# Farmadupe/vid_dup_finder_lib

Hardware: AMD Instinct MI355X
Metric: hash-pairs/sec all-pairs Hamming (search(), tolerance 0.35) [+ frames/sec DCT-hash in 'summary.hash_summary'] (higher is better)
Workload: dtype fp4 e2m1 ({0,1}) x fp4 -> f32 accumulate (exact half-integers < 2^11)

## Files before the change

### vid_dup_finder_lib_amd/csrc/api.cpp

```cpp
#include <algorithm>
#include <chrono>
#include <cmath>
#include <cstdio>
#include <cstdlib>
#include <cstring>
#include <memory>
#include <numeric>

#include "host_sort.h"
#include "vdf_ctx.h"

namespace {
thread_local std::string g_create_error;
inline double now_ms() { return std::chrono::duration<double, std::milli>(std::chrono::steady_clock::now().time_since_epoch()).count(); }
}

vdf_ctx::~vdf_ctx()
{
    if (!subs.empty() || !workers.empty()) vdf_impl::destroy_multi(this);
    if (copy_pool) vdf_impl::destroy_copy_pool(this);
    for (auto &kv : axis_tables) {
        kv.second->start.release(); kv.second->size.release(); kv.second->w.release();
        delete kv.second;
    }
    for (auto &kv : mfma_tables) {
        kv.second->operand.release(); kv.second->bias.release(); kv.second->meta.release();
        delete kv.second;
    }
    for (auto &kv : box_tables) {
        kv.second->blob.release(); kv.second->entries.release();
        delete kv.second;
    }
    DevBuf *all[] = {&row_lo, &row_hi, &tile_lo, &tile_hi, &tile_first, &tile_count, &tile_offset, &counters,
                     &hits, &perm, &matched, &exp_cols, &exp_rows, &pop_cols, &pop_rows, &cand, &group_cmin, &group_offset, &group_blocks, &up_hashes,
                     &up_dur, &up_ref_hashes, &up_ref_dur, &small, &frames, &frames2, &out_hashes, &out_hashes2, &out_dc,
                     &out_dc2, &cos_table, &crops, &crop_desc, &crop_tables, &crop_desc2, &crop_tables2, &crop_work, &sort_scratch, &sort_scratch_pub, &hits2, &hit_bitmaps, &bitmap_gather,
                     &out_zero, &out_zero2, &up_zero, &variant_hashes, &align_plan, &align_scratch, &align_up};
    for (DevBuf *b : all) b->release();
    for (PinBuf &b : pin) b.release();
    for (PinBuf &b : pin_out) b.release();
    pin_small.release();
    pin_ctrl.release();
    pin_crops.release();
    pin_desc.release();
    host_hits.buf.release();
    if (ev0) (void)hipEventDestroy(ev0);
    if (ev1) (void)hipEventDestroy(ev1);
    if (ev_mid) (void)hipEventDestroy(ev_mid);
    if (ev_wait) (void)hipEventDestroy(ev_wait);
    for (hipEvent_t e : ev_copy) if (e) (void)hipEventDestroy(e);
    for (hipEvent_t e : ev_done) if (e) (void)hipEventDestroy(e);
    if (copy_stream) (void)hipStreamDestroy(copy_stream);
    if (stream) (void)hipStreamDestroy(stream);
}

namespace vdf_impl {

// ... 89 lines not shown
    L.prune_step = 16;
    if (ctx->mfma_prune_step >= 0) {
        L.prune_step = ctx->mfma_prune_step;
    } else {
        for (int st = 6; st <= 14; st++) {
            const double bits = 64.0 * (st + 1);
            if (bits / 2 - 2.0 * std::sqrt(bits) >= (double)tol_int + 1) { L.prune_step = st; break; }
        }
    }
    if (mfma) L.prune_step = L.prune_step <= 6 ? 6 : L.prune_step <= 8 ? 8 : L.prune_step <= 10 ? 10 : L.prune_step <= 14 ? L.prune_step : 16;
    else L.prune_step = L.prune_step <= 6 ? 6 : L.prune_step <= 10 ? 10 : L.prune_step <= 12 ? 12 : 16;
    if (mfma) {
        L.group_size = std::min<uint32_t>(ctx->mfma_group, L.n_row_tiles);
        L.n_groups = (L.n_row_tiles + L.group_size - 1) / L.group_size;
        if (L.n_groups > 1024) return fail(ctx, VDF_E_INVAL, "too many row-tile groups");
        VDF_HIP(ctx, ctx->group_cmin.reserve((size_t)L.n_groups * 4));
        VDF_HIP(ctx, ctx->group_offset.reserve(((size_t)L.n_groups + 1) * 4));
        VDF_HIP(ctx, ctx->group_blocks.reserve((size_t)L.n_groups * 4));
        L.group_blocks = ctx->group_blocks.as<uint32_t>();
        L.group_cmin = ctx->group_cmin.as<uint32_t>();
        L.group_offset = ctx->group_offset.as<uint32_t>();
        const uint32_t k_steps = (uint32_t)(L.prune_step < 15 ? L.prune_step + 1 : 16);
        const uint32_t col_pad = (uint32_t)((n_cols + vdf::kMfmaRowPad - 1) / vdf::kMfmaRowPad * vdf::kMfmaRowPad) + vdf::kMfmaColPad;
        VDF_HIP(ctx, ctx->exp_cols.reserve((size_t)col_pad * 512));
        VDF_HIP(ctx, ctx->pop_cols.reserve((size_t)col_pad * 12));
        const ExpOwner want_owner{d_col_hashes, n_cols, k_steps, ctx->exp_cols.p};
        const bool reuse = ctx->pinned_db == d_col_hashes && ctx->pinned_n == n_cols && ctx->exp_owner == want_owner;
        if (!reuse) {
            ctx->exp_owner = ExpOwner{};
            VDF_HIP(ctx, vdf::launch_expand_fp4(L.col_hashes, (uint32_t)n_cols, col_pad, ctx->exp_cols.p, k_steps,
                                                ctx->pop_cols.as<float>(), stream));
            ctx->exp_owner = want_owner;
        }
        L.col_exp = ctx->exp_cols.p;
        L.col_pop3 = ctx->pop_cols.as<float>();
        L.col_pad = col_pad;
        if (d_row_hashes == d_col_hashes) {
            L.row_exp = ctx->exp_cols.p;
            L.row_pop3 = L.col_pop3;
            L.row_pad = col_pad;
        } else {
            const uint32_t row_pad = (uint32_t)((padded_rows + 127) / 128 * 128);
            VDF_HIP(ctx, ctx->exp_rows.reserve((size_t)row_pad * 512));
            VDF_HIP(ctx, ctx->pop_rows.reserve((size_t)row_pad * 12));
            VDF_HIP(ctx, vdf::launch_expand_fp4(L.row_hashes, (uint32_t)n_rows, row_pad, ctx->exp_rows.p, k_steps,
                                                ctx->pop_rows.as<float>(), stream));
            L.row_exp = ctx->exp_rows.p;
            L.row_pop3 = ctx->pop_rows.as<float>();
            L.row_pad = row_pad;
        }
    }
    const unsigned long long init[8] = {0, 0, 0, 0, 0xFFFFFFFFull, 0, 0, 0};
    const bool pin_ok = ctx->pin_small.reserve(kPinSmallBytes) && ctx->pin_small.pinned;
    uint64_t spec = std::min<uint64_t>(capacity, std::max<uint64_t>(ctx->hits_guess + ctx->hits_guess / 4 + 1024, 8192));
    if (!pin_ok || spec * sizeof(vdf_hit) > kPinSmallBytes) spec = 0;
    const bool spec_sort = spec && ctx->hits_guess >= kSpecSortHits;
    if (spec_sort) VDF_HIP(ctx, hipMemsetAsync(ctx->hits.p, 0xFF, (size_t)spec * sizeof(vdf_hit), stream));
    const bool adapt_refs = mode == 1 && mfma && ctx->mfma_chunk_cols == 0;
    if (adapt_refs && ctx->refs_hint_cols == n_cols && ctx->refs_hint_rows == n_rows && ctx->refs_hint_chunk) L.chunk_cols = ctx->refs_hint_chunk;
    if (!ctx->pin_ctrl.reserve(256)) return fail(ctx, VDF_E_OOM, "pinned staging");
    unsigned long long *pre = ctx->pin_ctrl.as<unsigned long long>() + 8;
    uint32_t total_tiles = 0;
    unsigned long long unsorted = 0, admitted = 0;
    for (int pass = 0;; pass++) {
        VDF_HIP(ctx, hipMemcpyAsync(ctx->counters.p, init, sizeof init, hipMemcpyHostToDevice, stream));
        VDF_HIP(ctx, vdf::launch_windows_tiles(mode, d_col_dur, (uint32_t)n_cols, d_row_dur, d_row_perm, (uint32_t)n_rows,
                                               row_begin, row_end, shard_index, shard_count, L, stream));
        VDF_HIP(ctx, hipMemcpyAsync(pre, L.counters, 64, hipMemcpyDeviceToHost, stream));
        VDF_HIP(ctx, hipMemcpyAsync(pre + 8, mfma ? L.group_offset + L.n_groups : L.tile_offset + L.n_row_tiles, 4,
                                    hipMemcpyDeviceToHost, stream));
        VDF_HIP(ctx, hipMemcpyAsync(pre + 9, L.tile_offset + L.n_row_tiles, 4, hipMemcpyDeviceToHost, stream));
        VDF_HIP(ctx, hipStreamSynchronize(stream));
// ... 2117 lines not shown
```

### vid_dup_finder_lib_amd/csrc/hamming.hip

```cpp
#include <algorithm>

#include "vdf_internal.h"

namespace vdf {

constexpr uint32_t kMaxBlocksPerLaunch = 4u << 20;

typedef const __attribute__((address_space(4))) uint32_t *const_u32_ptr;

__device__ __forceinline__ uint32_t sat_u32(double x)
{
    if (!(x == x)) return 0u;
    if (x <= 0.0) return 0u;
    if (x >= 4294967295.0) return 0xFFFFFFFFu;
    return (uint32_t)x;
}

__device__ __forceinline__ uint32_t partition_point_lt(const uint32_t *__restrict__ d, uint32_t n, uint32_t v)
{
    uint32_t lo = 0, hi = n;
    while (lo < hi) {
        uint32_t mid = lo + ((hi - lo) >> 1);
        if (d[mid] < v) lo = mid + 1; else hi = mid;
    }
// ... 255 lines not shown
#pragma unroll
            for (int k = 1; k < R; k++) m = min(m, d[k]);
        }
        if (__builtin_amdgcn_ballot_w64(m <= tol) != 0ull) {
            bool col_ok = true;
            if (matched) col_ok = ((((const_u32_ptr)(uintptr_t)matched)[c >> 5] >> (c & 31)) & 1u) == 0u;
            if (col_ok) {
#pragma unroll
                for (int k = 0; k < R; k++)
                    wave_append_hits(d[k] <= tol && c >= rlo[k] && c < rhi[k], rid[k], c, hits, capacity, counters, overflow_row);
            }
        }
    }
    if (threadIdx.x == 0) atomicAdd(&counters[1], (unsigned long long)(c_end - c_begin) * TILE_ROWS);
    if (CHKW < 32 && lane == 0 && n_early) atomicAdd(&counters[3], (unsigned long long)n_early * (64u * R));
}

typedef int v8i __attribute__((ext_vector_type(8)));
typedef int v4i __attribute__((ext_vector_type(4)));
typedef float v16f __attribute__((ext_vector_type(16)));

__global__ __launch_bounds__(256) void expand_fp4_kernel(const uint32_t *__restrict__ packed, uint32_t n,
                                                        uint32_t n_pad, uint4 *__restrict__ expanded,
                                                        uint32_t k_steps, float *__restrict__ pop,
                                                        float *__restrict__ popk, float *__restrict__ popkT)
{
    for (size_t idx = (size_t)blockIdx.x * 256 + threadIdx.x; idx < (size_t)n_pad * 32;
         idx += (size_t)gridDim.x * 256) {
    const uint32_t hsh = (uint32_t)(idx >> 5), dw = (uint32_t)idx & 31u;
    uint4 out = {0u, 0u, 0u, 0u};
    uint32_t w = 0;
    if (hsh < n) {
        w = packed[idx];
        uint32_t o[4];
#pragma unroll
        for (int j = 0; j < 4; j++) {
            uint32_t x = (w >> (8 * j)) & 0xFFu;
            x = (x | (x << 12)) & 0x000F000Fu;
            x = (x | (x << 6)) & 0x03030303u;
            x = (x | (x << 3)) & 0x11111111u;
            o[j] = x << 1;
        }
        out = make_uint4(o[0], o[1], o[2], o[3]);
    }
    expanded[idx] = out;
    if (pop) {
        uint32_t pc = (uint32_t)__builtin_popcount(w), pk = (dw & 15u) < k_steps ? pc : 0u;
#pragma unroll
        for (int o = 16; o > 0; o >>= 1) { pc += (uint32_t)__shfl_xor((int)pc, o, 32); pk += (uint32_t)__shfl_xor((int)pk, o, 32); }
        if (dw == 0) {
            pop[hsh] = (float)pc;
            popk[hsh] = (float)pk;
            popkT[(size_t)(hsh >> 7) * 128 + (hsh & 31u) * 4 + ((hsh >> 5) & 3u)] = (float)pk;
        }
    }
    }
}

template <int N>
struct IntC { static constexpr int value = N; };
template <int I, int N, class F>
__device__ __forceinline__ void static_for(F &&f)
{
    if constexpr (I < N) {
        f(IntC<I>{});
        static_for<I + 1, N>(f);
    }
}

struct CandEntry {
    uint32_t row_base;
    uint32_t col;
    uint32_t mask;
    uint32_t pad;
};

__global__ __launch_bounds__(256) void resolve_candidates_kernel(
    const CandEntry *__restrict__ cand, const unsigned long long *__restrict__ cand_head, uint32_t cand_capacity,
// ... 68 lines not shown
            if (bal == 0ull) continue;
            const uint32_t cnt = (uint32_t)__builtin_popcountll(bal);
            if (staged + cnt > kStage) flush();
            if (hit) {
                vdf_hit hp; hp.row = row_index_base + src; hp.col = ce.col;
                s_stage[wave][staged + __builtin_amdgcn_mbcnt_hi((uint32_t)(bal >> 32), __builtin_amdgcn_mbcnt_lo((uint32_t)bal, 0u))] = hp;
            }
            staged += cnt;
        }
    }
    flush();
}

template <int CHK, int WAVES>
__global__ __launch_bounds__(64 * WAVES, 2) void hamming_mfma2_kernel(
    const uint4 *__restrict__ row_exp, const uint32_t *__restrict__ row_perm, uint32_t n_rows,
    uint32_t row_index_base, const uint4 *__restrict__ col_exp, const uint32_t *__restrict__ row_lo,
    const uint32_t *__restrict__ row_hi, const uint32_t *__restrict__ tile_lo, const uint32_t *__restrict__ tile_hi,
    const uint32_t *__restrict__ tile_first, const uint32_t *__restrict__ tile_count,
    const uint32_t *__restrict__ group_offset, const uint32_t *__restrict__ group_cmin, uint32_t n_groups,
    uint32_t group_size, uint32_t shard_index, uint32_t shard_count, uint32_t n_row_tiles, uint32_t chunk_cols,
    uint32_t tol, const uint32_t *__restrict__ matched, int self_mode, vdf_hit *__restrict__ hits,
    unsigned long long capacity, unsigned long long *__restrict__ counters, uint32_t *__restrict__ overflow_row,
    uint32_t block_base, const float *__restrict__ row_pop3, uint32_t row_pad, const float *__restrict__ col_pop3,
    uint32_t col_pad, CandEntry *__restrict__ cand, uint32_t cand_capacity, unsigned long long *__restrict__ cand_head)
{
    constexpr int K = CHK < 15 ? CHK + 1 : 16;
    constexpr bool kRowcLds = K > 13;
    constexpr uint32_t kSub = WAVES >= 8 ? 4 : 2;
    constexpr uint32_t kColStep = 32 * kSub;
    constexpr int NBLK = 2 * (int)kSub;
    constexpr int NM = NBLK * K;
    constexpr int P = (K == 16 && WAVES >= 8) ? 2 : 4, NB = P + 1;
    constexpr uint32_t kTileRows = 64 * WAVES;
    constexpr int kDmaPerWave = (int)(kColStep * 32 / (64 * WAVES));
    constexpr int kDmaEvery = NM / kDmaPerWave;
    static_assert(kDmaEvery >= 2, "stage too short for its DMA pieces");
    constexpr int kTestAt = 2;
    static_assert(K >= kTestAt + 4, "block too short to hide the previous block's test");
    const uint32_t bid = blockIdx.x + block_base;
    __shared__ __attribute__((aligned(16))) uint4 s_b0[kColStep * 32];
    __shared__ __attribute__((aligned(16))) uint4 s_b1[kColStep * 32];
    const uint32_t tid = threadIdx.x, lane = tid & 63, g = lane >> 5, c31 = lane & 31;
    const uint32_t wave = (uint32_t)__builtin_amdgcn_readfirstlane((int)(tid >> 6));

    const_u32_ptr goff = (const_u32_ptr)(uintptr_t)group_offset;
    uint32_t gl = 0, gh = n_groups;
    while (gh - gl > 1) {
        const uint32_t mid = (gl + gh) >> 1;
        if (goff[mid] <= bid) gl = mid; else gh = mid;
    }
    const uint32_t idx = bid - goff[gl];
    const uint32_t per_group = (group_size + shard_count - 1) / shard_count;
    const uint32_t g0 = gl * group_size;
    const uint32_t t0 = g0 + (shard_index + shard_count - g0 % shard_count) % shard_count;
    const uint32_t t = t0 + (idx % per_group) * shard_count;
    const uint32_t chunk = ((const_u32_ptr)(uintptr_t)group_cmin)[gl] + idx / per_group;
    if (t >= n_row_tiles || t >= g0 + group_size) return;
    {
        const uint32_t f = ((const_u32_ptr)(uintptr_t)tile_first)[t], cnt = ((const_u32_ptr)(uintptr_t)tile_count)[t];
        if (chunk < f || chunk >= f + cnt) return;
    }
    const uint32_t t_lo = ((const_u32_ptr)(uintptr_t)tile_lo)[t];
    const uint32_t t_hi = ((const_u32_ptr)(uintptr_t)tile_hi)[t];
    const uint32_t c_begin = max(chunk * chunk_cols, t_lo);
    const uint32_t c_end = min((chunk + 1) * chunk_cols, t_hi);
    if (c_begin >= c_end) return;

    const float tol_f = (float)min(tol, 1024u);
    const float *row_popk = row_pop3 + row_pad;
    const float *col_popkT = col_pop3 + 2 * (size_t)col_pad;
    const uint32_t row0 = t * kTileRows + wave * 64;
    v4i a[2][K];
    const float4 *s_rc = nullptr;
    v16f rowc[2];
    uint32_t live[2];
#pragma unroll
    for (int rt = 0; rt < 2; rt++) {
        live[rt] = 0;
        const uint32_t p = row0 + 32 * rt + c31;
        uint32_t src = p;
        if (p < n_rows && row_perm) src = row_perm[p];
        const uint4 *rp = row_exp + (size_t)src * 32 + 16 * g;
#pragma unroll
        for (int s = 0; s < K; s++) {
            const uint4 v = rp[s];
            a[rt][s] = (v4i){(int)v.x, (int)v.y, (int)v.z, (int)v.w};
        }
#pragma unroll
        for (int r = 0; r < 16; r++) {
            const uint32_t pr = row0 + 32 * rt + (r & 3) + 8 * (r >> 2) + 4 * g;
            const uint32_t sr = (pr < n_rows && row_perm) ? row_perm[pr] : pr;
            rowc[rt][r] = -0.5f * row_popk[sr];
            if (row_hi[pr] > row_lo[pr]) live[rt] |= 1u << r;
        }
    }
    if constexpr (kRowcLds) {
        __shared__ __attribute__((aligned(16))) float4 s_rowc[WAVES * 2 * 2 * 4];
        float4 *mine = s_rowc + ((size_t)wave * 2 * 2 + g) * 4;
        if (c31 == 0) {
#pragma unroll
            for (int rt = 0; rt < 2; rt++)
#pragma unroll
                for (int q = 0; q < 4; q++)
                    mine[rt * 2 * 4 + q] = float4{rowc[rt][4 * q], rowc[rt][4 * q + 1], rowc[rt][4 * q + 2], rowc[rt][4 * q + 3]};
        }
        s_rc = mine;
    }
    const uint32_t cb0 = c_begin & ~(kColStep - 1);
    constexpr uint32_t kColsPerRound = 2 * WAVES;
    constexpr int kOffsets = 32 / kColsPerRound;
    static_assert(kOffsets >= 1 && (kOffsets & (kOffsets - 1)) == 0, "piece addressing");
    const uint32_t c0 = 2 * wave + g;
    uint32_t lane_off[kOffsets];
#pragma unroll
    for (int j = 0; j < kOffsets; j++) lane_off[j] = c0 * 512u + ((((lane & 31) ^ c0) << 4) ^ (16u * kColsPerRound * j));
    auto stage_rsrc = [&](uint32_t cb) __attribute__((always_inline)) {
        return __builtin_amdgcn_make_buffer_rsrc(
            const_cast<char *>(reinterpret_cast<const char *>(col_exp) + (size_t)cb * 512), 0, kColStep * 512u, 0x00020000);
    };
    auto load_piece = [&](__amdgpu_buffer_rsrc_t rs, uint4 *dst, int i) __attribute__((always_inline)) {
        auto *lds = (__attribute__((address_space(3))) void *)&dst[64 * WAVES * i + 64 * wave];
        const int voff = (int)lane_off[i & (kOffsets - 1)], soff = (int)(512u * kColsPerRound * (uint32_t)i);
        __builtin_amdgcn_raw_ptr_buffer_load_lds(rs, lds, 16, voff, soff, 0, 0);
    };
    auto load_thr = [&](uint32_t cb, float (&out)[kSub]) __attribute__((always_inline)) {
        const float *q = col_popkT + (size_t)(cb >> 7) * 128 + c31 * 4 + ((cb >> 5) & 3u);
        if constexpr (kSub == 4) {
            const float4 v = *reinterpret_cast<const float4 *>(q);
            out[0] = v.x; out[1] = v.y; out[2] = v.z; out[3] = v.w;
        } else {
            const float2 v = *reinterpret_cast<const float2 *>(q);
            out[0] = v.x; out[1] = v.y;
        }
    };

    v16f acc[2] = {v16f{}, v16f{}};
    if constexpr (kRowcLds) acc[0] = rowc[0];
    uint32_t n_early = 0;
    float thr[kSub], thr_next[kSub];

    constexpr uint32_t kCandChunk = 8, kCandChunkMax = 512;
    uint32_t q_chunk = kCandChunk, q_taken = 0;
    unsigned long long q_next = 0, q_end = 0;
    auto emit = [&](const v16f &c, float thrv, uint32_t live_rows, uint32_t rows_first, uint32_t col_first) __attribute__((always_inline)) {
        uint32_t mask = 0;
#pragma unroll
        for (int r = 0; r < 16; r++) mask |= (c[r] >= thrv) ? (1u << r) : 0u;
        mask &= live_rows;
        const uint32_t j = col_first + c31;
        if (j < c_begin || j >= c_end) mask = 0;
        const unsigned long long bal = __builtin_amdgcn_ballot_w64(mask != 0u);
        if (bal == 0ull) return;
        const uint32_t need = (uint32_t)__builtin_popcountll(bal);
        if (q_next + need > q_end) {
            if (q_taken >= 2) q_chunk = min(2u * q_chunk, kCandChunkMax);
            q_taken++;
            const uint32_t take = max((need + kCandChunk - 1) / kCandChunk * kCandChunk, q_chunk);
            unsigned long long base = 0;
            if (lane == 0) base = atomicAdd(cand_head, (unsigned long long)take);
            q_next = ((unsigned long long)(uint32_t)__builtin_amdgcn_readfirstlane((int)(base >> 32)) << 32) |
                     (uint32_t)__builtin_amdgcn_readfirstlane((int)(uint32_t)base);
            q_end = q_next + take;
        }
        const unsigned long long slot = q_next + __builtin_amdgcn_mbcnt_hi((uint32_t)(bal >> 32), __builtin_amdgcn_mbcnt_lo((uint32_t)bal, 0u));
        if (mask != 0u) {
            if (slot < cand_capacity) {
                CandEntry ce; ce.row_base = rows_first + 4 * g; ce.col = j; ce.mask = mask; ce.pad = 0;
                *reinterpret_cast<uint4 *>(&cand[slot]) = *reinterpret_cast<const uint4 *>(&ce);
            } else {
                const uint32_t p = rows_first + 4 * g + (uint32_t)(__builtin_ctz(mask) & 3) + 8 * (uint32_t)(__builtin_ctz(mask) >> 2);
                if (p < n_rows) atomicMin(overflow_row, row_index_base + (row_perm ? row_perm[p] : p));
            }
        }
        q_next += need;
    };

    auto run_stage = [&](uint32_t cb, const uint4 *cur, uint4 *nxt) __attribute__((always_inline)) {
        const uint32_t cb_next = cb + kColStep < c_end ? cb + kColStep : cb;
        const __amdgpu_buffer_rsrc_t rs_next = stage_rsrc(cb_next);
        load_thr(cb_next, thr_next);
        uint32_t flags = 0;
        uint4 fq[NB];
        auto frag = [&](int i) __attribute__((always_inline)) {
            const uint32_t sub = (uint32_t)((i / K) >> 1), s = (uint32_t)(i % K);
            return cur[((32u * sub + c31) << 5) | ((s + 16u * g) ^ c31)];
        };
#pragma unroll
        for (int i = 0; i < P; i++) fq[i] = frag(i);
        __builtin_amdgcn_sched_barrier(0);
        float m0 = 0.f, m1 = 0.f, m2 = 0.f, m3 = 0.f, m4 = 0.f, m5 = 0.f;
        static_for<0, NM>([&](auto ic) __attribute__((always_inline)) {
            constexpr int i = decltype(ic)::value;
            constexpr int blk = i / K, s = i % K, rt = blk & 1;
            const uint4 bv = fq[i % NB];
            const v8i b = {(int)bv.x, (int)bv.y, (int)bv.z, (int)bv.w, 0, 0, 0, 0};
            const v8i ar = {a[rt][s].x, a[rt][s].y, a[rt][s].z, a[rt][s].w, 0, 0, 0, 0};
            if constexpr (s == 0 && !kRowcLds) acc[rt] = __builtin_amdgcn_mfma_scale_f32_32x32x64_f8f6f4(ar, b, rowc[rt], 4, 4, 0, 0, 0, 0);
            else acc[rt] = __builtin_amdgcn_mfma_scale_f32_32x32x64_f8f6f4(ar, b, acc[rt], 4, 4, 0, 0, 0, 0);
            if constexpr (i + P < NM) fq[(i + P) % NB] = frag(i + P);
            if constexpr ((i % kDmaEvery) == 1 && (i / kDmaEvery) < kDmaPerWave) load_piece(rs_next, nxt, i / kDmaEvery);
            if constexpr (blk >= 1) {
                const v16f &c = acc[rt ^ 1];
                if constexpr (s == kTestAt) {
                    m0 = fmaxf(fmaxf(c[0], c[1]), c[2]); m1 = fmaxf(fmaxf(c[3], c[4]), c[5]); m2 = fmaxf(fmaxf(c[6], c[7]), c[8]);
                } else if constexpr (s == kTestAt + 1) {
                    m3 = fmaxf(fmaxf(c[9], c[10]), c[11]); m4 = fmaxf(fmaxf(c[12], c[13]), c[14]);
                } else if constexpr (s == kTestAt + 2) {
                    m5 = fmaxf(fmaxf(m0, m1), m2); m3 = fmaxf(fmaxf(m3, m4), c[15]);
                } else if constexpr (s == kTestAt + 3) {
                    if (__builtin_amdgcn_ballot_w64(fmaxf(m5, m3) >= thr[(blk - 1) >> 1]) != 0ull) {
                        flags |= 1u << (blk - 1);
                        emit(c, thr[(blk - 1) >> 1], live[rt ^ 1], row0 + 32u * (uint32_t)(rt ^ 1), cb + 32u * (uint32_t)((blk - 1) >> 1));
                    }
                }
            }
            if constexpr (kRowcLds && s >= kTestAt + 4 && s < kTestAt + 8) {
                constexpr int q = s - (kTestAt + 4);
                const float4 v = s_rc[((rt ^ 1) * 2) * 4 + q];
                acc[rt ^ 1][4 * q + 0] = v.x; acc[rt ^ 1][4 * q + 1] = v.y; acc[rt ^ 1][4 * q + 2] = v.z; acc[rt ^ 1][4 * q + 3] = v.w;
            }
            __builtin_amdgcn_sched_barrier(0);
        });
        {
            const v16f &c = acc[(NBLK - 1) & 1];
            m0 = fmaxf(fmaxf(c[0], c[1]), c[2]); m1 = fmaxf(fmaxf(c[3], c[4]), c[5]); m2 = fmaxf(fmaxf(c[6], c[7]), c[8]);
            m3 = fmaxf(fmaxf(c[9], c[10]), c[11]); m4 = fmaxf(fmaxf(c[12], c[13]), c[14]);
            const float pm = fmaxf(fmaxf(fmaxf(m0, m1), m2), fmaxf(fmaxf(m3, m4), c[15]));
            if (__builtin_amdgcn_ballot_w64(pm >= thr[kSub - 1]) != 0ull) {
                flags |= 1u << (NBLK - 1);
                emit(c, thr[kSub - 1], live[(NBLK - 1) & 1], row0 + 32u * (uint32_t)((NBLK - 1) & 1), cb + 32u * (kSub - 1));
            }
        }
        uint32_t valid = 0;
#pragma unroll
        for (uint32_t sub = 0; sub < kSub; sub++)
            if (cb + 32u * sub < c_end) valid |= 3u << (2 * sub);
        flags &= valid;
        n_early += (uint32_t)__builtin_popcount(valid & ~flags);
        asm volatile("s_waitcnt vmcnt(0)" ::: "memory");
        __syncthreads();
#pragma unroll
        for (uint32_t sub = 0; sub < kSub; sub++) thr[sub] = 0.5f * (thr_next[sub] - tol_f);
    };

#pragma unroll
    for (int i = 0; i < kDmaPerWave; i++) load_piece(stage_rsrc(cb0), s_b0, i);
    load_thr(cb0, thr_next);
#pragma unroll
    for (int rt = 0; rt < 2; rt++)
#pragma unroll
        for (int s = 0; s < K; s++) asm volatile("" ::"v"(a[rt][s]));
    asm volatile("s_waitcnt vmcnt(0)" ::: "memory");
    __syncthreads();
#pragma unroll
    for (uint32_t sub = 0; sub < kSub; sub++) thr[sub] = 0.5f * (thr_next[sub] - tol_f);
    for (uint32_t cb = cb0; cb < c_end; cb += 2 * kColStep) {
        run_stage(cb, s_b0, s_b1);
        if (cb + kColStep >= c_end) break;
        run_stage(cb + kColStep, s_b1, s_b0);
    }
    if (tid == 0) atomicAdd(&counters[1], (unsigned long long)(c_end - c_begin) * kTileRows);
    if (CHK < 15 && lane == 0 && n_early) atomicAdd(&counters[3], (unsigned long long)n_early * (32u * 32u));
}

__global__ __launch_bounds__(256) void hits_mark_incoming_kernel(const vdf_hit *__restrict__ hits, unsigned long long n,
                                                                 uint32_t *__restrict__ has_in)
{
    for (size_t i = (size_t)blockIdx.x * 256 + threadIdx.x; i < n; i += (size_t)gridDim.x * 256) {
        const uint32_t j = hits[i].col;
        if (!((has_in[j >> 5] >> (j & 31)) & 1u)) atomicOr(&has_in[j >> 5], 1u << (j & 31));
    }
}

__global__ __launch_bounds__(256) void hits_mark_covered_kernel(const vdf_hit *__restrict__ hits, unsigned long long n,
                                                                const uint32_t *__restrict__ has_in, uint32_t *__restrict__ covered)
{
    for (size_t i = (size_t)blockIdx.x * 256 + threadIdx.x; i < n; i += (size_t)gridDim.x * 256) {
        const vdf_hit h = hits[i];
// ... 147 lines not shown
                d += __builtin_popcount(v.x ^ hi[4 * q]) + __builtin_popcount(v.y ^ hi[4 * q + 1]) +
                     __builtin_popcount(v.z ^ hi[4 * q + 2]) + __builtin_popcount(v.w ^ hi[4 * q + 3]);
            }
            best = max(best, d);
        }
    }
    best = wave_max(best);
    if ((threadIdx.x & 63) == 0) s_max[threadIdx.x >> 6] = best;
    __syncthreads();
    if (threadIdx.x == 0) out[g] = max(max(s_max[0], s_max[1]), max(s_max[2], s_max[3]));
}

hipError_t launch_group_max_distance(const uint32_t *hashes, const unsigned long long *offsets,
                                     const unsigned long long *members, const uint32_t *ref_hashes,
                                     const long long *ref_index, uint32_t n_groups, uint32_t *out, hipStream_t stream)
{
    if (n_groups == 0) return hipSuccess;
    hipLaunchKernelGGL(group_max_distance_kernel, dim3(n_groups), dim3(256), 0, stream, hashes, offsets, members,
                       ref_hashes, ref_index, out);
    return hipGetLastError();
}

hipError_t launch_expand_fp4(const uint32_t *packed, uint32_t n, uint32_t n_pad, void *expanded, uint32_t k_steps,
                             float *pop3 , hipStream_t stream)
{
    if (n_pad == 0) return hipSuccess;
    if (pop3 && (n_pad % 128u)) return hipErrorInvalidValue;
    const size_t total = (size_t)n_pad * 32;
    hipLaunchKernelGGL(expand_fp4_kernel, dim3((uint32_t)std::min<size_t>((total + 255) / 256, kMaxBlocksPerLaunch)), dim3(256), 0, stream, packed, n, n_pad,
                       reinterpret_cast<uint4 *>(expanded), k_steps, pop3, pop3 ? pop3 + n_pad : nullptr,
                       pop3 ? pop3 + 2 * (size_t)n_pad : nullptr);
    return hipGetLastError();
}

hipError_t launch_hamming_tiles_mfma2(const SearchLaunch &L, uint32_t total_tiles, hipStream_t stream)
{
    if (total_tiles == 0) return hipSuccess;
    if (L.tile_rows != 512 && L.tile_rows != 256) return hipErrorInvalidValue;
    for (uint32_t base = 0; base < total_tiles; base += kMaxBlocksPerLaunch) {
        const uint32_t nb = std::min(kMaxBlocksPerLaunch, total_tiles - base);
#define VDF_MFMA2_LAUNCH(CK, WV)                                                                                    \
    hipLaunchKernelGGL((hamming_mfma2_kernel<CK, WV>), dim3(nb), dim3(64 * WV), 0, stream,                           \
                       reinterpret_cast<const uint4 *>(L.row_exp), L.row_perm, L.n_rows, L.row_index_base,           \
                       reinterpret_cast<const uint4 *>(L.col_exp), L.row_lo, L.row_hi, L.tile_lo, L.tile_hi,         \
                       L.tile_first, L.tile_count, L.group_offset, L.group_cmin, L.n_groups, L.group_size,           \
                       L.shard_index, L.shard_count, L.n_row_tiles, L.chunk_cols, L.tol, L.matched, L.self_mode,     \
                       L.hits, L.capacity, L.counters, L.overflow_row, base, L.row_pop3, L.row_pad, L.col_pop3, L.col_pad,                   \
                       reinterpret_cast<CandEntry *>(L.cand), L.cand_capacity, L.cand_head)
#define VDF_MFMA2_STEPS(WV)                                                                                         \
    switch (L.prune_step) {                                    \
    case 0: case 1: case 2: case 3: case 4: case 5: case 6: VDF_MFMA2_LAUNCH(6, WV); break;                          \
    case 7: case 8: VDF_MFMA2_LAUNCH(8, WV); break;                                                                  \
    case 9: case 10: VDF_MFMA2_LAUNCH(10, WV); break;                                                                \
    case 11: VDF_MFMA2_LAUNCH(11, WV); break;                                                                        \
    case 12: VDF_MFMA2_LAUNCH(12, WV); break;                                                                        \
    case 13: VDF_MFMA2_LAUNCH(13, WV); break;                                                                        \
    case 14: VDF_MFMA2_LAUNCH(14, WV); break;                                                                        \
    default: VDF_MFMA2_LAUNCH(16, WV); break;                                                                        \
    }
        if (L.tile_rows == 512) { VDF_MFMA2_STEPS(8) } else { VDF_MFMA2_STEPS(4) }
#undef VDF_MFMA2_STEPS
#undef VDF_MFMA2_LAUNCH
        hipError_t e = hipGetLastError();
        if (e != hipSuccess) return e;
    }
    return hipSuccess;
}

hipError_t launch_resolve_candidates(const SearchLaunch &L, hipStream_t stream)
{
// ... 8 lines not shown
```

### vid_dup_finder_lib_amd/csrc/vdf_ctx.h

```cpp
#pragma once
#include <condition_variable>
#include <functional>
#include <map>
#include <mutex>
#include <string>
#include <thread>
#include <vector>

#include "resize_tables.h"
#include <atomic>

#include "vdf_internal.h"

inline std::atomic<long long> g_live_device_bytes{0};
inline std::atomic<long long> g_live_pinned_bytes{0};

struct DevBuf {
    void *p = nullptr;
    size_t cap = 0;
    hipError_t reserve(size_t bytes)
    {
        if (bytes <= cap) return hipSuccess;
        release();
        size_t want = bytes + bytes / 8 + 256;
// ... 114 lines not shown
    size_t refs_hint_cols = 0, refs_hint_rows = 0;
    uint32_t refs_hint_chunk = 0;
    bool no_hit_filter = false;
    uint64_t hits_guess = 0;
    PinBuf pin_small;
    std::map<uint32_t, DeviceAxisTable *> axis_tables;
    std::map<uint64_t, DeviceMfmaTable *> mfma_tables;
    std::map<uint64_t, BoxTableSet *> box_tables;
    std::map<uint32_t, bool> axis_symmetric;
    bool no_device_path_order = false;
    bool lb_host_plan = false;
    bool no_lb_fused = false;
    int hash_no_persistent = 0, hash_wgs_per_cu = 3;
    bool hash_wgs_per_cu_set = false;
    uint32_t mfma_chunk_cols = 0, mfma_group = 8192;
    DevBuf group_cmin, group_offset, group_blocks;
    uint32_t mfma_min_wgs = 8192;
    uint64_t cand_scale = 1;
    uint32_t cand_capacity_override = 0;
    uint32_t mfma_self_rows = 512;
    uint32_t mfma_refs_rows = 256;
    int mfma_prune_step = -1;
    int search_backend = 1;
    DevBuf exp_cols, exp_rows, pop_cols, pop_rows, cand;
    size_t cand_dirty = SIZE_MAX;
    int wavestream_knob = 0;
    bool no_rowcrop = false, rowcrop_all = false, no_boxstream = false;
    bool no_smallcrop = false;
    int lb_side_strips = 0;
    int copy_threads = 0;
    size_t host_chunk_bytes = 32u << 20;
    bool host_direct = true;
    bool force_rccl = false;
    bool test_exchange_fail = false;
    bool err_secondary = false;
    int resize_mode = 0;
    struct HostHits {
        PinBuf buf;
        size_t size() const { return buf.cap / sizeof(vdf_hit); }
        bool resize(size_t n) { return buf.reserve(n * sizeof(vdf_hit)); }
        vdf_hit *data() const { return buf.as<vdf_hit>(); }
    } host_hits;
    vdf_impl::CopyPool *copy_pool = nullptr;
    uint64_t r_n_hits = 0;
    uint32_t r_overflow = 0xFFFFFFFFu;
    int r_rc = 0;

// ... 77 lines not shown
```

### vid_dup_finder_lib_amd/csrc/vdf_internal.h

```cpp
#pragma once
#include <hip/hip_runtime.h>
#include <stdint.h>

#include "../../include/vdf.h"
#include "hash_variant.h"
#include "resize_dispatch.h"
#include "windows_plan.h"
#include "align_plan.h"

namespace vdf {

constexpr int kDefaultRowsPerLane = 2;
constexpr uint32_t kDefaultChunkCols = 2048;

struct SearchLaunch {
    const uint32_t *row_hashes;
    const uint32_t *row_perm;
    uint32_t n_rows;
    uint32_t row_index_base;
    const uint32_t *col_hashes;
    uint32_t n_cols;
    const void *row_exp, *col_exp;
    const float *row_pop3 = nullptr, *col_pop3 = nullptr;
    uint32_t row_pad = 0, col_pad = 0;
    void *cand = nullptr;
    uint32_t cand_capacity = 0;
    unsigned long long *cand_head = nullptr;
    uint32_t *row_lo, *row_hi;
    uint32_t *tile_lo, *tile_hi, *tile_first, *tile_count, *tile_offset;
    uint32_t *group_cmin, *group_offset, *group_blocks;
    int prune_step = 16;
    uint32_t shard_index = 0, shard_count = 1;
    uint32_t n_groups, group_size;
    uint32_t n_row_tiles;
    uint32_t tile_rows;
    uint32_t chunk_cols;
    uint32_t tol;
    const uint32_t *matched;
    int self_mode;
    vdf_hit *hits;
    unsigned long long capacity;
    unsigned long long *counters;
    uint32_t *overflow_row;
};

hipError_t launch_windows_tiles(int mode, const uint32_t *col_dur, uint32_t n_cols, const uint32_t *row_dur,
                                const uint32_t *row_perm, uint32_t n_rows, uint32_t row_begin, uint32_t row_end,
                                uint32_t shard_index, uint32_t shard_count, const SearchLaunch &L,
                                hipStream_t stream);
hipError_t launch_hamming_tiles(const SearchLaunch &L, uint32_t total_tiles, hipStream_t stream);
constexpr uint32_t kMfmaRowPad = 512, kMfmaColPad = 128;
hipError_t launch_expand_fp4(const uint32_t *packed, uint32_t n, uint32_t n_pad, void *expanded, uint32_t k_steps,
                             float *pop3, hipStream_t stream);
hipError_t launch_hamming_tiles_mfma2(const SearchLaunch &L, uint32_t total_tiles, hipStream_t stream);
hipError_t launch_resolve_candidates(const SearchLaunch &L, hipStream_t stream);
hipError_t launch_filter_mark_incoming(const vdf_hit *hits, unsigned long long n_hits, uint32_t n_entries, uint32_t *bitmaps, hipStream_t stream);
hipError_t launch_filter_mark_covered(const vdf_hit *hits, unsigned long long n_hits, uint32_t n_entries, uint32_t *bitmaps, hipStream_t stream);
hipError_t launch_filter_compact(const vdf_hit *hits, unsigned long long n_hits, uint32_t n_entries, const uint32_t *bitmaps, vdf_hit *out,
                                 unsigned long long *counter, hipStream_t stream);
hipError_t launch_bitmap_or(uint32_t *dst, const uint32_t *srcs, size_t n_words, uint32_t n_srcs, hipStream_t stream);
hipError_t launch_group_max_distance(const uint32_t *hashes, const unsigned long long *offsets,
                                     const unsigned long long *members, const uint32_t *ref_hashes,
                                     const long long *ref_index, uint32_t n_groups, uint32_t *out, hipStream_t stream);

struct ResizeAxisTable {
    const int32_t *start;
    const int32_t *size;
    const int16_t *w;
    int32_t window;
    int32_t precision;
};

hipError_t launch_resize_generic(const uint8_t *frames, size_t n_clips, uint32_t w, uint32_t h, size_t frame_stride,
                                 size_t clip_stride, ResizeAxisTable th, ResizeAxisTable tv, int need_h, int need_v,
                                 int32_t y_first, int32_t tmp_rows, uint8_t *small, hipStream_t stream);
struct MfmaResizeArgs {
// ... 121 lines not shown
```

Measured before the change: 4669 billion.

## Pack only needed K-steps and popcount into compact per-hash fp4 image

The expanded fp4 hash image now stores only the K slots actually used per half (stride 2K+1) instead of a fixed 32 slots, with the popcount folded into a trailing pad slot rather than separate pop arrays. The MFMA kernel stages the smaller contiguous image into LDS via buffer-to-LDS pieces, reads column popcounts from LDS for thresholds instead of a separate global load, and drops the XOR swizzle addressing. This cuts global-to-LDS traffic and LDS footprint for pruned K, at the risk of LDS bank conflicts from the odd stride.

```diff
diff --git a/vid_dup_finder_lib_amd/csrc/api.cpp b/vid_dup_finder_lib_amd/csrc/api.cpp
--- a/vid_dup_finder_lib_amd/csrc/api.cpp
+++ b/vid_dup_finder_lib_amd/csrc/api.cpp
@@ -32,7 +32,7 @@
         delete kv.second;
     }
     DevBuf *all[] = {&row_lo, &row_hi, &tile_lo, &tile_hi, &tile_first, &tile_count, &tile_offset, &counters,
-                     &hits, &perm, &matched, &exp_cols, &exp_rows, &pop_cols, &pop_rows, &cand, &group_cmin, &group_offset, &group_blocks, &up_hashes,
+                     &hits, &perm, &matched, &exp_cols, &exp_rows, &cand, &group_cmin, &group_offset, &group_blocks, &up_hashes,
                      &up_dur, &up_ref_hashes, &up_ref_dur, &small, &frames, &frames2, &out_hashes, &out_hashes2, &out_dc,
                      &out_dc2, &cos_table, &crops, &crop_desc, &crop_tables, &crop_desc2, &crop_tables2, &crop_work, &sort_scratch, &sort_scratch_pub, &hits2, &hit_bitmaps, &bitmap_gather,
                      &out_zero, &out_zero2, &up_zero, &variant_hashes, &align_plan, &align_scratch, &align_up};
@@ -168,32 +168,23 @@
         L.group_offset = ctx->group_offset.as<uint32_t>();
         const uint32_t k_steps = (uint32_t)(L.prune_step < 15 ? L.prune_step + 1 : 16);
         const uint32_t col_pad = (uint32_t)((n_cols + vdf::kMfmaRowPad - 1) / vdf::kMfmaRowPad * vdf::kMfmaRowPad) + vdf::kMfmaColPad;
-        VDF_HIP(ctx, ctx->exp_cols.reserve((size_t)col_pad * 512));
-        VDF_HIP(ctx, ctx->pop_cols.reserve((size_t)col_pad * 12));
+        const size_t img_bytes = vdf::fp4img::hash_bytes(k_steps);
+        VDF_HIP(ctx, ctx->exp_cols.reserve((size_t)col_pad * img_bytes));
         const ExpOwner want_owner{d_col_hashes, n_cols, k_steps, ctx->exp_cols.p};
         const bool reuse = ctx->pinned_db == d_col_hashes && ctx->pinned_n == n_cols && ctx->exp_owner == want_owner;
         if (!reuse) {
             ctx->exp_owner = ExpOwner{};
-            VDF_HIP(ctx, vdf::launch_expand_fp4(L.col_hashes, (uint32_t)n_cols, col_pad, ctx->exp_cols.p, k_steps,
-                                                ctx->pop_cols.as<float>(), stream));
+            VDF_HIP(ctx, vdf::launch_expand_fp4(L.col_hashes, (uint32_t)n_cols, col_pad, ctx->exp_cols.p, k_steps, stream));
             ctx->exp_owner = want_owner;
         }
         L.col_exp = ctx->exp_cols.p;
-        L.col_pop3 = ctx->pop_cols.as<float>();
-        L.col_pad = col_pad;
         if (d_row_hashes == d_col_hashes) {
             L.row_exp = ctx->exp_cols.p;
-            L.row_pop3 = L.col_pop3;
-            L.row_pad = col_pad;
         } else {
             const uint32_t row_pad = (uint32_t)((padded_rows + 127) / 128 * 128);
-            VDF_HIP(ctx, ctx->exp_rows.reserve((size_t)row_pad * 512));
-            VDF_HIP(ctx, ctx->pop_rows.reserve((size_t)row_pad * 12));
-            VDF_HIP(ctx, vdf::launch_expand_fp4(L.row_hashes, (uint32_t)n_rows, row_pad, ctx->exp_rows.p, k_steps,
-                                                ctx->pop_rows.as<float>(), stream));
+            VDF_HIP(ctx, ctx->exp_rows.reserve((size_t)row_pad * img_bytes));
+            VDF_HIP(ctx, vdf::launch_expand_fp4(L.row_hashes, (uint32_t)n_rows, row_pad, ctx->exp_rows.p, k_steps, stream));
             L.row_exp = ctx->exp_rows.p;
-            L.row_pop3 = ctx->pop_rows.as<float>();
-            L.row_pad = row_pad;
         }
     }
     const unsigned long long init[8] = {0, 0, 0, 0, 0xFFFFFFFFull, 0, 0, 0};
diff --git a/vid_dup_finder_lib_amd/csrc/fp4_image.h b/vid_dup_finder_lib_amd/csrc/fp4_image.h
--- /dev/null
+++ b/vid_dup_finder_lib_amd/csrc/fp4_image.h
@@ -0,0 +1,46 @@
+#pragma once
+#include <stdint.h>
+
+namespace vdf {
+namespace fp4img {
+
+constexpr uint32_t kSlotBytes = 16;
+constexpr uint32_t kPieceSlots = 64;
+constexpr uint32_t kLdsBytes = 160u * 1024u;
+constexpr int kInstantiatedK[8] = {7, 9, 11, 12, 13, 14, 15, 16};
+
+constexpr uint32_t stride(uint32_t K) { return 2 * K + 1; }
+constexpr uint32_t pad_slot(uint32_t K) { return 2 * K; }
+constexpr uint32_t hash_bytes(uint32_t K) { return stride(K) * kSlotBytes; }
+constexpr int slot(uint32_t K, uint32_t dword)
+{
+    return dword < K ? (int)dword : (dword >= 16 && dword < 16 + K) ? (int)(K + dword - 16) : -1;
+}
+constexpr uint32_t dword_of_slot(uint32_t K, uint32_t s) { return s < K ? s : 16 + (s - K); }
+constexpr uint32_t frag_slot(uint32_t K, uint32_t col, uint32_t s, uint32_t g) { return col * stride(K) + s + K * g; }
+
+constexpr uint32_t stage_slots(uint32_t col_step, uint32_t K) { return col_step * stride(K); }
+constexpr uint32_t stage_bytes(uint32_t col_step, uint32_t K) { return stage_slots(col_step, K) * kSlotBytes; }
+constexpr uint32_t pieces(uint32_t col_step, uint32_t K) { return stage_slots(col_step, K) / kPieceSlots; }
+constexpr uint32_t piece_of(uint32_t wave, uint32_t i, uint32_t waves) { return waves * i + wave; }
+constexpr uint32_t wave_pieces(uint32_t col_step, uint32_t K, uint32_t waves, uint32_t wave)
+{
+    return wave < pieces(col_step, K) ? (pieces(col_step, K) - wave + waves - 1) / waves : 0;
+}
+constexpr uint32_t max_wave_pieces(uint32_t col_step, uint32_t K, uint32_t waves) { return wave_pieces(col_step, K, waves, 0); }
+
+constexpr uint32_t col_step(uint32_t waves) { return waves >= 8 ? 128 : 64; }
+constexpr bool rowc_in_lds(uint32_t K) { return K > 13; }
+constexpr uint32_t rowc_bytes(uint32_t K, uint32_t waves) { return rowc_in_lds(K) ? waves * 2 * 2 * 4 * 16 : 0; }
+constexpr uint32_t kernel_lds_bytes(uint32_t K, uint32_t waves) { return 2 * stage_bytes(col_step(waves), K) + rowc_bytes(K, waves); }
+
+constexpr uint8_t kReadB128Groups[4][16] = {
+    {0, 1, 2, 3, 12, 13, 14, 15, 20, 21, 22, 23, 24, 25, 26, 27},
+    {4, 5, 6, 7, 8, 9, 10, 11, 16, 17, 18, 19, 28, 29, 30, 31},
+    {32, 33, 34, 35, 44, 45, 46, 47, 52, 53, 54, 55, 56, 57, 58, 59},
+    {36, 37, 38, 39, 40, 41, 42, 43, 48, 49, 50, 51, 60, 61, 62, 63},
+};
+constexpr uint32_t bank_group(uint32_t byte_addr) { return (byte_addr / 16) % 16; }
+
+}
+}
diff --git a/vid_dup_finder_lib_amd/csrc/hamming.hip b/vid_dup_finder_lib_amd/csrc/hamming.hip
--- a/vid_dup_finder_lib_amd/csrc/hamming.hip
+++ b/vid_dup_finder_lib_amd/csrc/hamming.hip
@@ -301,15 +301,16 @@
 
 __global__ __launch_bounds__(256) void expand_fp4_kernel(const uint32_t *__restrict__ packed, uint32_t n,
                                                         uint32_t n_pad, uint4 *__restrict__ expanded,
-                                                        uint32_t k_steps, float *__restrict__ pop,
-                                                        float *__restrict__ popk, float *__restrict__ popkT)
-{
+                                                        uint32_t k_steps)
+{
+    const uint32_t stride = fp4img::stride(k_steps);
     for (size_t idx = (size_t)blockIdx.x * 256 + threadIdx.x; idx < (size_t)n_pad * 32;
          idx += (size_t)gridDim.x * 256) {
     const uint32_t hsh = (uint32_t)(idx >> 5), dw = (uint32_t)idx & 31u;
+    const int sl = fp4img::slot(k_steps, dw);
     uint4 out = {0u, 0u, 0u, 0u};
     uint32_t w = 0;
-    if (hsh < n) {
+    if (hsh < n && sl >= 0) {
         w = packed[idx];
         uint32_t o[4];
 #pragma unroll
@@ -322,17 +323,12 @@
         }
         out = make_uint4(o[0], o[1], o[2], o[3]);
     }
-    expanded[idx] = out;
-    if (pop) {
-        uint32_t pc = (uint32_t)__builtin_popcount(w), pk = (dw & 15u) < k_steps ? pc : 0u;
-#pragma unroll
-        for (int o = 16; o > 0; o >>= 1) { pc += (uint32_t)__shfl_xor((int)pc, o, 32); pk += (uint32_t)__shfl_xor((int)pk, o, 32); }
-        if (dw == 0) {
-            pop[hsh] = (float)pc;
-            popk[hsh] = (float)pk;
-            popkT[(size_t)(hsh >> 7) * 128 + (hsh & 31u) * 4 + ((hsh >> 5) & 3u)] = (float)pk;
-        }
-    }
+    uint4 *img = expanded + (size_t)hsh * stride;
+    if (sl >= 0) img[sl] = out;
+    uint32_t pk = (uint32_t)__builtin_popcount(w);
+#pragma unroll
+    for (int o = 16; o > 0; o >>= 1) pk += (uint32_t)__shfl_xor((int)pk, o, 32);
+    if (dw == 0) img[fp4img::pad_slot(k_steps)] = make_uint4(__float_as_uint((float)pk), 0u, 0u, 0u);
     }
 }
 
@@ -447,25 +443,26 @@
     uint32_t group_size, uint32_t shard_index, uint32_t shard_count, uint32_t n_row_tiles, uint32_t chunk_cols,
     uint32_t tol, const uint32_t *__restrict__ matched, int self_mode, vdf_hit *__restrict__ hits,
     unsigned long long capacity, unsigned long long *__restrict__ counters, uint32_t *__restrict__ overflow_row,
-    uint32_t block_base, const float *__restrict__ row_pop3, uint32_t row_pad, const float *__restrict__ col_pop3,
-    uint32_t col_pad, CandEntry *__restrict__ cand, uint32_t cand_capacity, unsigned long long *__restrict__ cand_head)
+    uint32_t block_base, CandEntry *__restrict__ cand, uint32_t cand_capacity, unsigned long long *__restrict__ cand_head)
 {
     constexpr int K = CHK < 15 ? CHK + 1 : 16;
-    constexpr bool kRowcLds = K > 13;
-    constexpr uint32_t kSub = WAVES >= 8 ? 4 : 2;
-    constexpr uint32_t kColStep = 32 * kSub;
+    constexpr uint32_t kStride = fp4img::stride(K), kPad = fp4img::pad_slot(K);
+    constexpr bool kRowcLds = fp4img::rowc_in_lds(K);
+    constexpr uint32_t kColStep = fp4img::col_step(WAVES);
+    constexpr uint32_t kSub = kColStep / 32;
     constexpr int NBLK = 2 * (int)kSub;
     constexpr int NM = NBLK * K;
     constexpr int P = (K == 16 && WAVES >= 8) ? 2 : 4, NB = P + 1;
     constexpr uint32_t kTileRows = 64 * WAVES;
-    constexpr int kDmaPerWave = (int)(kColStep * 32 / (64 * WAVES));
+    constexpr uint32_t kPieces = fp4img::pieces(kColStep, K);
+    constexpr int kDmaPerWave = (int)fp4img::max_wave_pieces(kColStep, K, WAVES);
     constexpr int kDmaEvery = NM / kDmaPerWave;
     static_assert(kDmaEvery >= 2, "stage too short for its DMA pieces");
     constexpr int kTestAt = 2;
     static_assert(K >= kTestAt + 4, "block too short to hide the previous block's test");
     const uint32_t bid = blockIdx.x + block_base;
-    __shared__ __attribute__((aligned(16))) uint4 s_b0[kColStep * 32];
-    __shared__ __attribute__((aligned(16))) uint4 s_b1[kColStep * 32];
+    __shared__ __attribute__((aligned(16))) uint4 s_b0[fp4img::stage_slots(kColStep, K)];
+    __shared__ __attribute__((aligned(16))) uint4 s_b1[fp4img::stage_slots(kColStep, K)];
     const uint32_t tid = threadIdx.x, lane = tid & 63, g = lane >> 5, c31 = lane & 31;
     const uint32_t wave = (uint32_t)__builtin_amdgcn_readfirstlane((int)(tid >> 6));
 
@@ -493,8 +490,6 @@
     if (c_begin >= c_end) return;
 
     const float tol_f = (float)min(tol, 1024u);
-    const float *row_popk = row_pop3 + row_pad;
-    const float *col_popkT = col_pop3 + 2 * (size_t)col_pad;
     const uint32_t row0 = t * kTileRows + wave * 64;
     v4i a[2][K];
     const float4 *s_rc = nullptr;
@@ -506,7 +501,7 @@
         const uint32_t p = row0 + 32 * rt + c31;
         uint32_t src = p;
         if (p < n_rows && row_perm) src = row_perm[p];
-        const uint4 *rp = row_exp + (size_t)src * 32 + 16 * g;
+        const uint4 *rp = row_exp + fp4img::frag_slot(K, 0, 0, g) + (size_t)src * kStride;
 #pragma unroll
         for (int s = 0; s < K; s++) {
             const uint4 v = rp[s];
@@ -516,7 +511,7 @@
         for (int r = 0; r < 16; r++) {
             const uint32_t pr = row0 + 32 * rt + (r & 3) + 8 * (r >> 2) + 4 * g;
             const uint32_t sr = (pr < n_rows && row_perm) ? row_perm[pr] : pr;
-            rowc[rt][r] = -0.5f * row_popk[sr];
+            rowc[rt][r] = -0.5f * __uint_as_float(row_exp[(size_t)sr * kStride + kPad].x);
             if (row_hi[pr] > row_lo[pr]) live[rt] |= 1u << r;
         }
     }
@@ -533,37 +528,25 @@
         s_rc = mine;
     }
     const uint32_t cb0 = c_begin & ~(kColStep - 1);
-    constexpr uint32_t kColsPerRound = 2 * WAVES;
-    constexpr int kOffsets = 32 / kColsPerRound;
-    static_assert(kOffsets >= 1 && (kOffsets & (kOffsets - 1)) == 0, "piece addressing");
-    const uint32_t c0 = 2 * wave + g;
-    uint32_t lane_off[kOffsets];
-#pragma unroll
-    for (int j = 0; j < kOffsets; j++) lane_off[j] = c0 * 512u + ((((lane & 31) ^ c0) << 4) ^ (16u * kColsPerRound * j));
     auto stage_rsrc = [&](uint32_t cb) __attribute__((always_inline)) {
         return __builtin_amdgcn_make_buffer_rsrc(
-            const_cast<char *>(reinterpret_cast<const char *>(col_exp) + (size_t)cb * 512), 0, kColStep * 512u, 0x00020000);
+            const_cast<char *>(reinterpret_cast<const char *>(col_exp) + (size_t)cb * fp4img::hash_bytes(K)), 0,
+            fp4img::stage_bytes(kColStep, K), 0x00020000);
     };
-    auto load_piece = [&](__amdgpu_buffer_rsrc_t rs, uint4 *dst, int i) __attribute__((always_inline)) {
-        auto *lds = (__attribute__((address_space(3))) void *)&dst[64 * WAVES * i + 64 * wave];
-        const int voff = (int)lane_off[i & (kOffsets - 1)], soff = (int)(512u * kColsPerRound * (uint32_t)i);
-        __builtin_amdgcn_raw_ptr_buffer_load_lds(rs, lds, 16, voff, soff, 0, 0);
-    };
-    auto load_thr = [&](uint32_t cb, float (&out)[kSub]) __attribute__((always_inline)) {
-        const float *q = col_popkT + (size_t)(cb >> 7) * 128 + c31 * 4 + ((cb >> 5) & 3u);
-        if constexpr (kSub == 4) {
-            const float4 v = *reinterpret_cast<const float4 *>(q);
-            out[0] = v.x; out[1] = v.y; out[2] = v.z; out[3] = v.w;
-        } else {
-            const float2 v = *reinterpret_cast<const float2 *>(q);
-            out[0] = v.x; out[1] = v.y;
+    constexpr uint32_t kPieceBytes = fp4img::kPieceSlots * fp4img::kSlotBytes;
+    const uint32_t lane_off = kPieceBytes * fp4img::piece_of(wave, 0, WAVES) + lane * fp4img::kSlotBytes;
+    auto load_piece = [&](__amdgpu_buffer_rsrc_t rs, uint4 *dst, auto ic) __attribute__((always_inline)) {
+        constexpr uint32_t i = (uint32_t)decltype(ic)::value, first = fp4img::piece_of(0, i, WAVES);
+        if (first + WAVES <= kPieces || wave < kPieces - first) {
+            auto *lds = (__attribute__((address_space(3))) void *)&dst[fp4img::kPieceSlots * first + fp4img::kPieceSlots * wave];
+            __builtin_amdgcn_raw_ptr_buffer_load_lds(rs, lds, 16, (int)lane_off, (int)(kPieceBytes * first), 0, 0);
         }
     };
 
     v16f acc[2] = {v16f{}, v16f{}};
     if constexpr (kRowcLds) acc[0] = rowc[0];
     uint32_t n_early = 0;
-    float thr[kSub], thr_next[kSub];
+    float thr[kSub];
 
     constexpr uint32_t kCandChunk = 8, kCandChunkMax = 512;
     uint32_t q_chunk = kCandChunk, q_taken = 0;
@@ -604,15 +587,18 @@
     auto run_stage = [&](uint32_t cb, const uint4 *cur, uint4 *nxt) __attribute__((always_inline)) {
         const uint32_t cb_next = cb + kColStep < c_end ? cb + kColStep : cb;
         const __amdgpu_buffer_rsrc_t rs_next = stage_rsrc(cb_next);
-        load_thr(cb_next, thr_next);
         uint32_t flags = 0;
         uint4 fq[NB];
         auto frag = [&](int i) __attribute__((always_inline)) {
             const uint32_t sub = (uint32_t)((i / K) >> 1), s = (uint32_t)(i % K);
-            return cur[((32u * sub + c31) << 5) | ((s + 16u * g) ^ c31)];
+            return cur[fp4img::frag_slot(K, 32u * sub + c31, s, g)];
         };
 #pragma unroll
         for (int i = 0; i < P; i++) fq[i] = frag(i);
+        float pbk[kSub];
+#pragma unroll
+        for (uint32_t sub = 0; sub < kSub; sub++)
+            pbk[sub] = *reinterpret_cast<const float *>(&cur[(32u * sub + c31) * kStride + kPad]);
         __builtin_amdgcn_sched_barrier(0);
         float m0 = 0.f, m1 = 0.f, m2 = 0.f, m3 = 0.f, m4 = 0.f, m5 = 0.f;
         static_for<0, NM>([&](auto ic) __attribute__((always_inline)) {
@@ -624,7 +610,11 @@
             if constexpr (s == 0 && !kRowcLds) acc[rt] = __builtin_amdgcn_mfma_scale_f32_32x32x64_f8f6f4(ar, b, rowc[rt], 4, 4, 0, 0, 0, 0);
             else acc[rt] = __builtin_amdgcn_mfma_scale_f32_32x32x64_f8f6f4(ar, b, acc[rt], 4, 4, 0, 0, 0, 0);
             if constexpr (i + P < NM) fq[(i + P) % NB] = frag(i + P);
-            if constexpr ((i % kDmaEvery) == 1 && (i / kDmaEvery) < kDmaPerWave) load_piece(rs_next, nxt, i / kDmaEvery);
+            if constexpr ((i % kDmaEvery) == 1 && (i / kDmaEvery) < kDmaPerWave) load_piece(rs_next, nxt, IntC<i / kDmaEvery>{});
+            if constexpr (i == K - 1) {
+#pragma unroll
+                for (uint32_t sub = 0; sub < kSub; sub++) thr[sub] = fmaf(0.5f, pbk[sub], -0.5f * tol_f);
+            }
             if constexpr (blk >= 1) {
                 const v16f &c = acc[rt ^ 1];
                 if constexpr (s == kTestAt) {
@@ -665,21 +655,15 @@
         n_early += (uint32_t)__builtin_popcount(valid & ~flags);
         asm volatile("s_waitcnt vmcnt(0)" ::: "memory");
         __syncthreads();
-#pragma unroll
-        for (uint32_t sub = 0; sub < kSub; sub++) thr[sub] = 0.5f * (thr_next[sub] - tol_f);
     };
 
-#pragma unroll
-    for (int i = 0; i < kDmaPerWave; i++) load_piece(stage_rsrc(cb0), s_b0, i);
-    load_thr(cb0, thr_next);
+    static_for<0, kDmaPerWave>([&](auto ic) __attribute__((always_inline)) { load_piece(stage_rsrc(cb0), s_b0, ic); });
 #pragma unroll
     for (int rt = 0; rt < 2; rt++)
 #pragma unroll
         for (int s = 0; s < K; s++) asm volatile("" ::"v"(a[rt][s]));
     asm volatile("s_waitcnt vmcnt(0)" ::: "memory");
     __syncthreads();
-#pragma unroll
-    for (uint32_t sub = 0; sub < kSub; sub++) thr[sub] = 0.5f * (thr_next[sub] - tol_f);
     for (uint32_t cb = cb0; cb < c_end; cb += 2 * kColStep) {
         run_stage(cb, s_b0, s_b1);
         if (cb + kColStep >= c_end) break;
@@ -873,14 +857,13 @@
 }
 
 hipError_t launch_expand_fp4(const uint32_t *packed, uint32_t n, uint32_t n_pad, void *expanded, uint32_t k_steps,
-                             float *pop3 , hipStream_t stream)
+                             hipStream_t stream)
 {
     if (n_pad == 0) return hipSuccess;
-    if (pop3 && (n_pad % 128u)) return hipErrorInvalidValue;
+    if ((n_pad % 128u) || k_steps < 1 || k_steps > 16) return hipErrorInvalidValue;
     const size_t total = (size_t)n_pad * 32;
     hipLaunchKernelGGL(expand_fp4_kernel, dim3((uint32_t)std::min<size_t>((total + 255) / 256, kMaxBlocksPerLaunch)), dim3(256), 0, stream, packed, n, n_pad,
-                       reinterpret_cast<uint4 *>(expanded), k_steps, pop3, pop3 ? pop3 + n_pad : nullptr,
-                       pop3 ? pop3 + 2 * (size_t)n_pad : nullptr);
+                       reinterpret_cast<uint4 *>(expanded), k_steps);
     return hipGetLastError();
 }
 
@@ -896,7 +879,7 @@
                        reinterpret_cast<const uint4 *>(L.col_exp), L.row_lo, L.row_hi, L.tile_lo, L.tile_hi,         \
                        L.tile_first, L.tile_count, L.group_offset, L.group_cmin, L.n_groups, L.group_size,           \
                        L.shard_index, L.shard_count, L.n_row_tiles, L.chunk_cols, L.tol, L.matched, L.self_mode,     \
-                       L.hits, L.capacity, L.counters, L.overflow_row, base, L.row_pop3, L.row_pad, L.col_pop3, L.col_pad,                   \
+                       L.hits, L.capacity, L.counters, L.overflow_row, base,                   \
                        reinterpret_cast<CandEntry *>(L.cand), L.cand_capacity, L.cand_head)
 #define VDF_MFMA2_STEPS(WV)                                                                                         \
     switch (L.prune_step) {                                    \
diff --git a/vid_dup_finder_lib_amd/csrc/vdf_ctx.h b/vid_dup_finder_lib_amd/csrc/vdf_ctx.h
--- a/vid_dup_finder_lib_amd/csrc/vdf_ctx.h
+++ b/vid_dup_finder_lib_amd/csrc/vdf_ctx.h
@@ -160,7 +160,7 @@
     uint32_t mfma_refs_rows = 256;
     int mfma_prune_step = -1;
     int search_backend = 1;
-    DevBuf exp_cols, exp_rows, pop_cols, pop_rows, cand;
+    DevBuf exp_cols, exp_rows, cand;
     size_t cand_dirty = SIZE_MAX;
     int wavestream_knob = 0;
     bool no_rowcrop = false, rowcrop_all = false, no_boxstream = false;
diff --git a/vid_dup_finder_lib_amd/csrc/vdf_internal.h b/vid_dup_finder_lib_amd/csrc/vdf_internal.h
--- a/vid_dup_finder_lib_amd/csrc/vdf_internal.h
+++ b/vid_dup_finder_lib_amd/csrc/vdf_internal.h
@@ -7,6 +7,7 @@
 #include "resize_dispatch.h"
 #include "windows_plan.h"
 #include "align_plan.h"
+#include "fp4_image.h"
 
 namespace vdf {
 
@@ -21,8 +22,6 @@
     const uint32_t *col_hashes;
     uint32_t n_cols;
     const void *row_exp, *col_exp;
-    const float *row_pop3 = nullptr, *col_pop3 = nullptr;
-    uint32_t row_pad = 0, col_pad = 0;
     void *cand = nullptr;
     uint32_t cand_capacity = 0;
     unsigned long long *cand_head = nullptr;
@@ -51,7 +50,7 @@
 hipError_t launch_hamming_tiles(const SearchLaunch &L, uint32_t total_tiles, hipStream_t stream);
 constexpr uint32_t kMfmaRowPad = 512, kMfmaColPad = 128;
 hipError_t launch_expand_fp4(const uint32_t *packed, uint32_t n, uint32_t n_pad, void *expanded, uint32_t k_steps,
-                             float *pop3, hipStream_t stream);
+                             hipStream_t stream);
 hipError_t launch_hamming_tiles_mfma2(const SearchLaunch &L, uint32_t total_tiles, hipStream_t stream);
 hipError_t launch_resolve_candidates(const SearchLaunch &L, hipStream_t stream);
 hipError_t launch_filter_mark_incoming(const vdf_hit *hits, unsigned long long n_hits, uint32_t n_entries, uint32_t *bitmaps, hipStream_t stream);
```

Measured after the change: 4653 billion. Within noise of the previous version (-0.3%).
